# yhtang/GraphDot

Measured on AMD Instinct MI355X. Metric: graph-pairs/sec (Gram matrix), higher is better.
Workload: dtype f64

## Files before the change

### graphdot_amd/csrc/device/mgk_oc.h

```cpp
#ifndef GRAPHDOT_HIP_MGK_OC_H_
#define GRAPHDOT_HIP_MGK_OC_H_
#include "mgk_solver.h"

#ifdef GD_STAMPS
#define GD_OC_STAMP(k) (st_t[k] = __builtin_amdgcn_s_memtime())
#else
#define GD_OC_STAMP(k) ((void)0)
#endif
#ifdef GD_MARKS
#define GD_MARK(name) asm volatile("; GDMARK " #name)
#else
#define GD_MARK(name) ((void)0)
#endif

namespace graphdot {
namespace mgk {

template<int DMAX> struct class_order {
    constexpr static int NC = DMAX + 1, NCP = NC * NC;
    unsigned char d1[NCP], d2[NCP];
    constexpr class_order() : d1{}, d2{} {
        int n = 0;
        for (int p = DMAX * DMAX; p >= 0; --p)
            for (int a = 0; a <= DMAX; ++a)
// ... 229 lines not shown
    }

    __device__ static __forceinline__ graph_header_t load_header(graph_header_t const *ptr, [[maybe_unused]] int &n_orig) {
        if constexpr (QUOT) {
            graph_header_t h = scalar_load(ptr);
            n_orig = (int)((unsigned)h.n_node >> 16);
            h.n_node &= 0xFFFF;
            return h;
        } else {
            return scalar_load(ptr);
        }
    }
    __device__ static __forceinline__ Graph view_graph(char const *image, graph_header_t const &h, [[maybe_unused]] int n_orig) {
        if constexpr (QUOT) return Graph::quotient(image, h, n_orig);
        else return Graph(image, h);
    }

    __device__ static __forceinline__ float cg_ratio(float a, float b) { return a / b; }
    __device__ static __forceinline__ double cg_ratio(double a, double b) {
        double y = __builtin_amdgcn_rcp(b);
        y = __builtin_fma(__builtin_fma(-b, y, 1.0), y, y);
        y = __builtin_fma(__builtin_fma(-b, y, 1.0), y, y);
        return a * y;
    }

    __device__ static __forceinline__ int row_pos(int k, int wv, int lane) {
        return k * T + 64 * ((k & 1) ? W - 1 - wv : wv) + lane;
    }

    struct row_t {
        int i1, i2, rs1, rs2, d1, d2, prod;
    };
    constexpr static int GQU = QUOT ? GU : 1, GQV = QUOT ? GV : 1;
    struct grid_t {
        unsigned a[GU], b[GV];
        unsigned j1[GU], j2[GV];
        unsigned t1[GU], t2[GV];
        bool u[GU], v[GV];
        int row;
    };

    __device__ static __forceinline__ void run(PF const &full, lds_t &lds, real *dyn) {
        P const &prm = common(full);
        const int lane = wave::laneid();
        const int tid = (W == 1) ? lane : (int)threadIdx.x;
        const int wv = (W == 1) ? 0 : uni((int)(threadIdx.x / 64));
        real *const lp = dyn;
        real *const lY = lp + (size_t)prm.u_capacity * C;
        unsigned *const rowmap = reinterpret_cast<unsigned *>(lY + (HAS_Y ? (size_t)Y_REALS : (size_t)0));
        char *const lG1 = reinterpret_cast<char *>(rowmap + NR);
        char *const lG2 = lG1 + prm.g_capacity;
        [[maybe_unused]] real *const lV = reinterpret_cast<real *>(lG2 + prm.g_capacity);
        real *const red0 = lds.red[0], *const red1 = lds.red[1];
        using reduce = alternating_reduce<real, W>;
        using sreduce = alternating_reduce<sreal, W>;
        sreal *const sred0 = reinterpret_cast<sreal *>(red0), *const sred1 = reinterpret_cast<sreal *>(red1);
        const unsigned lY_off = uni((int)lds_offset(lY));
        graph_header_t const *const headers = reinterpret_cast<graph_header_t const *>(prm.arena);
        const int dump = (int)prm.u_capacity - 1;

        if constexpr (DENSE) {
            if (prm.flags & F_DENSE) {
                for (unsigned k = tid; k < prm.u_capacity * (unsigned)C; k += T) lp[k] = real(0);
                job_sync<W>();
            }
        }
#ifdef GD_STAMPS
        unsigned long long st_t[6], st_acc[7] = {0, 0, 0, 0, 0, 0, 0};
#endif
        for (unsigned t = blockIdx.x; t < prm.n_launch_jobs; t += gridDim.x) {
            GD_OC_STAMP(0);
            const job_t job = scalar_load(prm.jobs + t);
            [[maybe_unused]] int no1 = 0, no2 = 0;
            graph_header_t h1 = load_header(headers + job.i, no1), h2 = load_header(headers + job.j, no2);
            if constexpr (ORIENT) {
                bool flip = false;
#pragma unroll
                for (int d = GV + 1; d <= DMAX; ++d) flip |= h2.hist[d] != 0;
                if (flip) {
                    const graph_header_t h = h1;
                    h1 = h2;
                    h2 = h;
                    const int no = no1;
                    no1 = no2;
                    no2 = no;
                }
            }
            const int n1 = h1.n_node, n2 = h2.n_node, N = n1 * n2;
            const int ldp = n2 | 1;
            const real q = prm.q, q0 = prm.q0;
            const real inv1q2 = real(1) / ((real(1) - q) * (real(1) - q));
            const real bscale = q * q / (q0 * q0);
            const unsigned nzpad1 = ((unsigned)n1 + 3u) & ~3u, nzpad2 = ((unsigned)n2 + 3u) & ~3u;
            const unsigned cb1 = TAB ? (nzpad1 + (((unsigned)h1.n_nz + 3u) & ~3u) + 15u) & ~15u : 0u;
            const unsigned cb2 = TAB ? (nzpad2 + (((unsigned)h2.n_nz + 3u) & ~3u) + 15u) & ~15u : 0u;

            GD_MARK(stage);
            job_sync<W>();
            {
                typedef unsigned v4 __attribute__((ext_vector_type(4)));
                const unsigned w1 = (h1.perm + 2u * n1 - h1.degree + cb1 + 15u) / 16u;
                const unsigned w2 = (h2.perm + 2u * n2 - h2.degree + cb2 + 15u) / 16u;
                const v4 *const s1 = reinterpret_cast<const v4 *>(prm.arena + h1.degree - cb1);
                const v4 *const s2 = reinterpret_cast<const v4 *>(prm.arena + h2.degree - cb2);
                v4 *const d1 = reinterpret_cast<v4 *>(lG1);
                v4 *const d2 = reinterpret_cast<v4 *>(lG2);
                constexpr int K = 2;
                const unsigned wmax = w1 > w2 ? w1 : w2;
#pragma nounroll
                for (unsigned base = 0; base < wmax; base += K * T) {
                    v4 v1[K], v2[K];
#pragma unroll
                    for (int k = 0; k < K; ++k) {
                        const unsigned w = base + k * T + tid;
                        v1[k] = w < w1 ? s1[w] : v4{0u, 0u, 0u, 0u};
                        v2[k] = w < w2 ? s2[w] : v4{0u, 0u, 0u, 0u};
                    }
#pragma unroll
                    for (int k = 0; k < K; ++k) {
                        const unsigned w = base + k * T + tid;
                        if (w < w1) d1[w] = v1[k];
                        if (w < w2) d2[w] = v2[k];
                    }
                }
                if constexpr (!STATIC && !FLY) {
#pragma unroll
                    for (int k = 0; k < R; ++k)
#pragma unroll
                        for (int c = 0; c < C; ++c) lY[(k * T + tid) * C + c] = 0;
                }
            }
            const Graph g1 = view_graph(lG1 + cb1 - h1.degree, h1, no1);
            const Graph g2 = view_graph(lG2 + cb2 - h2.degree, h2, no2);
            [[maybe_unused]] auto qweight = [](Graph const &g, nz_t z) -> real {
                return real(at32(g.scale, (unsigned)z.i)) * real(at32(g.scale, (unsigned)z.j));
            };
            std::uint8_t const *const ncls1 = reinterpret_cast<std::uint8_t const *>(lG1);
            std::uint8_t const *const ncls2 = reinterpret_cast<std::uint8_t const *>(lG2);
            std::uint8_t const *const ecls1 = ncls1 + nzpad1;
            std::uint8_t const *const ecls2 = ncls2 + nzpad2;
            const unsigned nvc = prm.n_vclass, nec = prm.n_eclass;
            real const *const kvtab = prm.tables;
            real const *const ketab = kvtab + nvc * nvc;
            real const *const dkvtab = ketab + nec * nec;
            real const *const dketab = dkvtab + (size_t)NodeK::jac_dims * nvc * nvc;
            auto kappa_v = [&](int i1, int i2, node_t const &v1, node_t const &v2) -> real {
                if constexpr (TAB) return at32(kvtab, __umul24((unsigned)ncls1[i1], nvc) + ncls2[i2]);
                else return real(prm.node_kernel(v1, v2));
            };
            std::uint16_t const *const lrp1 = g1.rowptr;
            std::uint16_t const *const lrp2 = g2.rowptr;
            job_sync<W>();

            [[maybe_unused]] bool dense_pair = false;
            [[maybe_unused]] edge_t *dE1 = nullptr, *dE2T = nullptr;
            if constexpr (DENSE) {
                const unsigned n2p = ((unsigned)n2 + 3u) & ~3u;
                const unsigned nn1 = (unsigned)n1 * (unsigned)n1, nn2 = EW * n2p * DSTRIDE;
                dense_pair = (prm.flags & F_DENSE) && n2 <= (int)DSTRIDE &&
                             23u * (unsigned)h1.n_nz * (unsigned)h2.n_nz > 9u * nn1 * (unsigned)n2 * (unsigned)n2;
                dE1 = reinterpret_cast<edge_t *>(lG2 + prm.g_capacity);
                dE2T = reinterpret_cast<edge_t *>(reinterpret_cast<char *>(dE1) + (nn1 * (unsigned)sizeof(edge_t) + 15u) / 16u * 16u);
                if (dense_pair) {
                    edge_t fill1 = at32(g1.edge, 0u), fill2 = at32(g2.edge, 0u);
                    fill1.weight = 0;
                    fill2.weight = 0;
                    unsigned fw[EW];
                    __builtin_memcpy(fw, &fill2, sizeof(edge_t));
                    unsigned *const planes = reinterpret_cast<unsigned *>(dE2T);
                    for (unsigned k = tid; k < nn1; k += T) dE1[k] = fill1;
                    for (unsigned k = tid; k < nn2; k += T) {
// ... 77 lines not shown
                r.rs2 = lrp2[r.i2];
                r.d1 = ok ? (int)lrp1[r.i1 + 1] - r.rs1 : 0;
                r.d2 = ok ? (int)lrp2[r.i2 + 1] - r.rs2 : 0;
                r.prod = r.d1 * r.d2;
                return r;
            };

            struct walk_t {
                unsigned e1, end1, last1, e2, rs2, end2;
                int row;
                __device__ __forceinline__ bool valid() const { return e1 < end1; }
                __device__ __forceinline__ unsigned a() const { return e1 < last1 ? e1 : last1; }
                __device__ __forceinline__ void next() {
                    ++e2;
                    const bool wrap = e2 == end2;
                    e2 = wrap ? rs2 : e2;
                    e1 += wrap ? 1u : 0u;
                }
            };
            auto open_walk = [&](int kb) -> walk_t {
                const row_t r = open_row(kb);
                const bool live = r.prod > 0;
                walk_t w;
                w.e1 = live ? (unsigned)r.rs1 : 0u;
                w.end1 = live ? (unsigned)(r.rs1 + r.d1) : 0u;
                w.last1 = live ? (unsigned)(r.rs1 + r.d1 - 1) : 0u;
                w.rs2 = live ? (unsigned)r.rs2 : 0u;
                w.end2 = live ? (unsigned)(r.rs2 + r.d2) : 1u;
                w.e2 = w.rs2;
                w.row = r.i1 * ldp + r.i2;
                return w;
            };

            auto open_grid = [&](unsigned base, unsigned elem) -> grid_t {
                const row_t r = open_row(0);
                const bool live = r.prod > 0;
                grid_t g;
                g.row = r.i1 * ldp + r.i2;
#pragma unroll
                for (int k = 0; k < GU; ++k) {
                    g.u[k] = k < r.d1;
                    if (k < GV) g.v[k] = k < r.d2;
                    g.a[k] = live ? (unsigned)r.rs1 + (g.u[k] ? (unsigned)k : 0u) : 0u;
                    if (k < GV) g.b[k] = live ? (unsigned)r.rs2 + (g.v[k] ? (unsigned)k : 0u) : 0u;
                    const nz_t z1 = at32(g1.nz, g.a[k]), z2 = at32(g2.nz, k < GV ? g.b[k] : 0u);
                    g.j1[k] = base + __umul24((unsigned)z1.j, (unsigned)ldp) * elem;
                    if (k < GV) g.j2[k] = (unsigned)z2.j * elem;
                    if constexpr (TAB) {
                        g.t1[k] = __umul24((unsigned)ecls1[g.a[k]], nec);
                        if (k < GV) g.t2[k] = (unsigned)ecls2[g.b[k]];
                    }
                }
                return g;
            };

            GD_MARK(slots);
            real val[SA];
            unsigned adr[NADR];
            const unsigned lp_off = lds_offset(lp);
            constexpr unsigned ELEM = CW * sizeof(real);
            unsigned fm[NM];
#pragma unroll
            for (int w = 0; w < NM; ++w) fm[w] = 0;
            int n_slots = 0;
            if constexpr (!FLY) {
                if constexpr (STATIC) {
#pragma unroll
                    for (int k = 0; k < R; ++k)
                        if (k * T < N) n_slots = LAY::T.end[k];
                } else {
#pragma unroll
                for (int k = 0; k < R; ++k) {
                    const int pos = row_pos(k, wv, 0);
                    int trip = 0;
                    if (pos < N) {
                        const unsigned rm = (unsigned)uni((int)rowmap[pos]);
                        const int i1 = (int)(rm >> 16), i2 = (int)(rm & 0xFFFFu);
                        trip = uni(((int)lrp1[i1 + 1] - (int)lrp1[i1]) * ((int)lrp2[i2 + 1] - (int)lrp2[i2]));
                    }
                    if (trip > 0) {
                        n_slots += trip;
                        const int last = n_slots - 1;
#pragma unroll
                        for (int w = 0; w < NM; ++w)
                            if (last / 32 == w) fm[w] |= 1u << (last % 32);
                    }
                }
                n_slots = n_slots > S ? S : n_slots;
                }
                if constexpr (ONE_PASS) {
                    int kb = 0;
                    walk_t cur = G0 ? walk_t{} : open_walk(0);
                    [[maybe_unused]] grid_t grid;
                    [[maybe_unused]] edge_t ge1[GU], ge2[GV];
                    [[maybe_unused]] real gw1[GQU], gw2[GQV];
                    if constexpr (G0 > 0) {
                        grid = open_grid(lp_off, ELEM);
                        if constexpr (QUOT) {
#pragma unroll
                            for (int k = 0; k < GU; ++k) {
                                gw1[k] = qweight(g1, at32(g1.nz, grid.a[k]));
                                if (k < GV) gw2[k] = qweight(g2, at32(g2.nz, grid.b[k]));
                            }
                        }
                        if constexpr (!TAB || (GD_WEIGHTED && edge_weight<edge_t>::value)) {
#pragma unroll
                            for (int k = 0; k < GU; ++k) {
                                ge1[k] = at32(g1.edge, grid.a[k]);
                                if (k < GV) ge2[k] = at32(g2.edge, grid.b[k]);
                            }
                        }
                    }
                    constexpr bool GPRE = QUOT && TAB && G0 > 0 &&
                        !(sizeof(real) == 8 && G0 == 16 && S == 20 && R == 2);
                    [[maybe_unused]] real gtab[GPRE ? G0 : 1];
                    if constexpr (GPRE) {
#pragma unroll
                        for (int s = 0; s < G0; ++s)
                            gtab[s] = at32(ketab, grid.t1[s / GV] + grid.t2[s % GV]);
                    }
    #pragma unroll
                    for (int s = 0; s < S; ++s) {
                        if (s % SETUP_CHUNK == 0) __builtin_amdgcn_sched_barrier(0);
                        if constexpr (GPRE) {
                            if (s < G0 && s % SETUP_CHUNK == 0) {
#pragma unroll
                                for (int u = s; u < s + SETUP_CHUNK && u < G0; ++u)
                                    asm volatile("" : "+v"(gtab[u]));
                            }
                        }
                        real e;
                        bool ok;
                        unsigned col;
                        if (s < G0) {
                            const int gu = s / GV, gv = s % GV;
                            ok = grid.u[gu] && grid.v[gv];
                            if constexpr (TAB) {
                                if constexpr (GPRE) e = gtab[s];
                                else e = at32(ketab, grid.t1[gu] + grid.t2[gv]);
                                if constexpr (GD_WEIGHTED && edge_weight<edge_t>::value)
                                    e *= real(edge_weight<edge_t>::get(ge1[gu])) *
                                         real(edge_weight<edge_t>::get(ge2[gv]));
                            } else {
                                e = prm.edge_kernel(ge1[gu], ge2[gv]);
                            }
                            if constexpr (QUOT) e *= gw1[gu] * gw2[gv];
                            col = ok ? grid.j1[gu] + grid.j2[gv] : lp_off;
                        } else {
                        ok = cur.valid();
                        const unsigned a = cur.a(), b = cur.e2;
                        const nz_t z1 = at32(g1.nz, a), z2 = at32(g2.nz, b);
                        if constexpr (TAB) {
                            e = at32(ketab, __umul24((unsigned)ecls1[a], nec) + ecls2[b]);
                            if constexpr (GD_WEIGHTED && edge_weight<edge_t>::value)
                                e *= real(edge_weight<edge_t>::get(at32(g1.edge, a))) *
                                     real(edge_weight<edge_t>::get(at32(g2.edge, b)));
                        } else {
                            const edge_t e1 = at32(g1.edge, a), e2 = at32(g2.edge, b);
                            e = prm.edge_kernel(e1, e2);
                        }
                        if constexpr (QUOT) e *= qweight(g1, z1) * qweight(g2, z2);
                        col = ok ? __umul24((unsigned)z1.j, (unsigned)ldp) + (unsigned)z2.j : 0u;
                        col = lp_off + col * ELEM;
                        }
                        if (SL > 0 && s >= SREG) {
                            lV[(s - SREG) * T + tid] = ok ? e : real(0);
                        } else {
                            val[s] = ok ? e : real(0);
                        }
                        if constexpr (PACK) {
                            if (s % 2 == 0) adr[s / 2] = col;
                            else adr[s / 2] |= col << 16;
                        } else {
                            adr[s] = col;
                        }
                        if (s % SETUP_CHUNK == SETUP_CHUNK - 1 || s == S - 1) {
#pragma unroll
                            for (int u = s - s % SETUP_CHUNK; u <= s; ++u) {
                                if (SL > 0 && u >= SREG) {
                                    if constexpr (PACK) asm volatile("" : "+v"(adr[u / 2]));
                                    else asm volatile("" : "+v"(adr[u]));
                                } else if constexpr (PACK) asm volatile("" : "+v"(val[u]), "+v"(adr[u / 2]));
                                else asm volatile("" : "+v"(val[u]), "+v"(adr[u]));
                            }
                        }
                        if (s >= G0) cur.next();
                        if (flush_at(s, fm) && s != S - 1) {
                            ++kb;
                            cur = open_walk(kb);
                        }
                    }
                } else {
                    int kb = 0, j = 0, ja = 0, jb = 0;
                    row_t cur = open_row(0);
                    [[maybe_unused]] unsigned ab_[PACK ? SA : 1];
                    unsigned (&ab)[PACK ? SA : NADR] = select_array<PACK>(ab_, adr);
    #pragma unroll
                    for (int s = 0; s < S; ++s) {
                        ab[s] = (s < n_slots && j < cur.prod)
                            ? ((unsigned)(cur.rs1 + ja) << 16) | (unsigned)(cur.rs2 + jb) : ~0u;
                        asm volatile("" : "+v"(ab[s]));
                        ++j;
                        ++jb;
                        if (jb >= cur.d2) {
                            jb = 0;
                            ++ja;
                        }
                        if ((fm[s / 32] >> (s % 32)) & 1u) {
                            ++kb;
// ... 1171 lines not shown
```

### graphdot_amd/csrc/gdhost.cpp

```cpp
#include "gdhost.h"
#include "gdquotient.h"

#include <algorithm>
#include <cstdlib>
#include <cstring>
#include <numeric>
#include <atomic>
#include <cmath>
#include <exception>
#include <mutex>
#include <thread>
#include <vector>

namespace {

constexpr int64_t ALIGN = 16;
inline int64_t pad(int64_t n) { return (n + ALIGN - 1) / ALIGN * ALIGN; }

struct rect_order_t {
    int a[256], b[256], prod[257];
    int n_upto[16], upto[16][256];
    rect_order_t() {
        int n = 0;
        for (int p = 15 * 15; p >= 0; --p)
// ... 568 lines not shown
        }
    const bool with_jobs = jobs && jobs_sorted;
    parallel_ranges(n_jobs, T, [&](int64_t t0, int64_t t1, int k) {
        std::vector<int64_t> &pos = start[(size_t)k];
        for (int64_t t = t0; t < t1; ++t) {
            const int64_t at = pos[rank[(size_t)t]]++;
            order[at] = (uint32_t)t;
            if (with_jobs) {
                jobs_sorted[2 * at] = jobs[2 * t];
                jobs_sorted[2 * at + 1] = jobs[2 * t + 1];
            }
        }
    });
    return 0;
} catch (...) { return -3; }

int gdh_gather_section(const uint8_t *blob, const int64_t *blob_off, const int64_t *sec_off,
                       int32_t col, const int64_t *count, int64_t G, int32_t itemsize,
                       uint8_t *out, int64_t out_bytes) try {
    if (G < 0 || col < 0 || col >= 6 || itemsize < 0) return -1;
    int64_t at = 0;
    for (int64_t g = 0; g < G; ++g) {
        const int64_t nb = count[g] * (int64_t)itemsize;
        if (nb < 0 || at + nb > out_bytes) return -2;
        std::memcpy(out + at, blob + blob_off[g] + sec_off[g * 6 + col], (size_t)nb);
        at += nb;
    }
    return 0;
} catch (...) { return -3; }

int gdh_assemble_arena(int64_t G, const uint8_t *blob, const int64_t *blob_off,
                       const int64_t *starts, const int64_t *cbytes, const int64_t *n_node,
                       const int64_t *n_nz, const uint8_t *ncls, const uint8_t *ecls,
                       uint8_t *host, int64_t host_bytes) try {
    if (G < 0) return -1;
    int64_t vn = 0, ve = 0;
    for (int64_t g = 0; g < G; ++g) {
        const int64_t nb = blob_off[g + 1] - blob_off[g];
        if (nb < 0 || starts[g] < cbytes[g] || starts[g] + nb > host_bytes) return -2;
        std::memcpy(host + starts[g], blob + blob_off[g], (size_t)nb);
        if (ncls && ecls && cbytes[g] > 0) {
            uint8_t *c0 = host + starts[g] - cbytes[g];
            const int64_t npad = (n_node[g] + 3) / 4 * 4;
            if (npad + n_nz[g] > cbytes[g]) return -2;
            std::memcpy(c0, ncls + vn, (size_t)n_node[g]);
            std::memcpy(c0 + npad, ecls + ve, (size_t)n_nz[g]);
        }
        vn += n_node[g];
        ve += n_nz[g];
    }
    return 0;
} catch (...) { return -3; }

int gdh_pairwise_jobs(int64_t nx, int64_t ny, uint32_t *jobs) try {
    if (nx < 0 || ny < -1 || nx + (ny > 0 ? ny : 0) > 0xFFFFFFFFll) return -1;
    int64_t t = 0;
    if (ny < 0) {
        for (int64_t i = 0; i < nx; ++i)
            for (int64_t j = i; j < nx; ++j, ++t) {
                jobs[2 * t] = (uint32_t)i;
                jobs[2 * t + 1] = (uint32_t)j;
            }
    } else {
        for (int64_t i = 0; i < nx; ++i)
            for (int64_t j = 0; j < ny; ++j, ++t) {
                jobs[2 * t] = (uint32_t)i;
                jobs[2 * t + 1] = (uint32_t)(nx + j);
            }
    }
    return 0;
} catch (...) { return -3; }

}
```

### graphdot_amd/hip/hostlib.py

```python
import ctypes
import os
import subprocess
import threading
import numpy as np

_HERE = os.path.dirname(os.path.abspath(__file__))
CSRC = os.path.join(os.path.dirname(_HERE), 'csrc')
INCLUDE = os.path.join(os.path.dirname(os.path.dirname(_HERE)), 'include')
LIB_PATH = os.path.join(CSRC, 'libgdhost.so')
_lock = threading.Lock()
_lib = None

_vp, _i32, _i64 = ctypes.c_void_p, ctypes.c_int32, ctypes.c_int64
SIGNATURES = {
    'gdh_pack_graphs': [_i32] + [_vp] * 7 + [_i32, _vp, _i32, _i32, _i32, _i32,
                                            _vp, _i64] + [_vp] * 10
    + [_i64, _vp, _vp],
    'gdh_number_records': [_vp, _i64, _i32, _vp, _vp, _i32, _vp, _vp, _vp],
    'gdh_classify_oc': [_i64] + [_vp] * 7 + [_i32] + [_vp] * 6
    + [_i32, _i32, _i64, _i32, _vp, _vp, _vp],
    'gdh_pair_keys': [_vp, _i64, _vp, _i32, _i32, _vp, _vp],
    'gdh_order_jobs': [_vp, _i64, _vp, _i64, _i64, _vp, _vp, _vp],
    'gdh_pairwise_jobs': [_i64, _i64, _vp],
    'gdh_gather_section': [_vp, _vp, _vp, _i32, _vp, _i64, _i32, _vp, _i64],
    'gdh_assemble_arena': [_i64] + [_vp] * 9 + [_i64],
    'gdh_quotient_graph': [_i32, _i32, _vp, _vp, _i32, _vp, _vp, _vp, _i32,
                           _vp, _vp, _i64, _vp, _vp],
}


class HostLibError(RuntimeError):
    pass


def build_library(force=False):
    src = os.path.join(CSRC, 'gdhost.cpp')
    hdrs = [os.path.join(INCLUDE, h) for h in ('gdhost.h', 'gdquotient.h')]
    if (not force and os.path.exists(LIB_PATH)
            and os.path.getmtime(LIB_PATH) >= max(
                os.path.getmtime(f) for f in [src] + hdrs)):
        return LIB_PATH
    cxx = os.environ.get('CXX', 'g++')
    tmp = LIB_PATH + f'.{os.getpid()}.tmp'
    cmd = [cxx, '-O2', '-fPIC', '-shared', '-std=c++17', '-pthread',
           f'-I{INCLUDE}', src,
           '-o', tmp]
    r = subprocess.run(cmd, capture_output=True, text=True)
    if r.returncode != 0:
        raise HostLibError(f'building libgdhost.so failed:\n{r.stderr}')
    os.replace(tmp, LIB_PATH)
    return LIB_PATH


def lib():
    global _lib
    with _lock:
        if _lib is None:
            L = ctypes.CDLL(build_library())
# ... 132 lines not shown
    raw = out = None
    if jobs is not None:
        jobs = np.ascontiguousarray(jobs)
        raw = jobs.view(np.uint32)
        out = np.empty_like(jobs)
    _check(lib().gdh_order_jobs(
        _p(pk), len(pk), _p(rank_of_key), len(rank_of_key), int(n_ranks),
        _p(order), _p(raw), None if out is None else _p(out.view(np.uint32))),
        'gdh_order_jobs')
    return order if jobs is None else (order, out)


def pairwise_jobs(nx, ny=None, dtype=None):
    n = nx * (nx + 1) // 2 if ny is None else nx * ny
    jobs = np.empty(2 * n, np.uint32)
    _check(lib().gdh_pairwise_jobs(int(nx), -1 if ny is None else int(ny),
                                   _p(jobs)), 'gdh_pairwise_jobs')
    return jobs if dtype is None else jobs.view(dtype)


def gather_section(blob, blob_off, sec_off, col, count, dtype):
    dtype = np.dtype(dtype)
    count = _c(count, np.int64)
    blob_off = _c(blob_off, np.int64)
    out = np.empty(int(count.sum()), dtype=dtype)
    raw = out.view(np.uint8) if dtype.itemsize else out
    _check(lib().gdh_gather_section(
        _p(blob), _p(blob_off), _p(_c(sec_off, np.int64)), int(col), _p(count),
        len(count), dtype.itemsize, _p(raw), out.nbytes), 'gdh_gather_section')
    return out


def assemble_arena(blob, blob_off, starts, cbytes, n_node, n_nz, ncls, ecls,
                   host):
    _check(lib().gdh_assemble_arena(
        len(starts), _p(blob), _p(_c(blob_off, np.int64)),
        _p(_c(starts, np.int64)), _p(_c(cbytes, np.int64)),
        _p(_c(n_node, np.int64)), _p(_c(n_nz, np.int64)),
        None if ncls is None else _p(_c(ncls, np.uint8)),
        None if ecls is None else _p(_c(ecls, np.uint8)),
        _p(host), host.nbytes), 'gdh_assemble_arena')


def quotient_graph(dg):
    n, nnz = int(dg.n_node), int(dg.n_nz)
    nsz, esz = np.dtype(dg.node_t).itemsize, np.dtype(dg.edge_t).itemsize
    o, src = dg.offsets, np.ascontiguousarray(dg.blob)
    base = src.ctypes.data

    def at(name):
        return ctypes.c_void_p(base + int(o[name]))
    cap = len(src) + 8 * n + 64
    blob = np.empty(cap, np.uint8)
    offs = np.zeros(7, np.int64)
    counts = np.zeros(3, np.int64)
    _check(lib().gdh_quotient_graph(
        n, nnz, at('degree'), at('node'), nsz, at('rowptr'), at('nz'),
        at('edge'), esz, at('perm'), _p(blob), cap, _p(offs), _p(counts)),
        'gdh_quotient_graph')
    return blob[:int(counts[2])], offs.tolist(), int(counts[0]), int(counts[1])


_collect = None


def collector():
    global _collect
    if _collect is None:
        with _lock:
            if _collect is None:
                _collect = _build_collector()
    return _collect

# ... 61 lines not shown
```

### graphdot_amd/kernel/marginalized/_backend_hip.py

```python
import copy
import os
import re
import uuid
import zlib
from collections import OrderedDict, namedtuple
import numpy as np
from ...codegen import Template
from ...util import gcpause
from ...util.cookie import IdentityCache
from ...codegen.sympy_printer import to_real_expr
from ...codegen.typetool import _dtype_util
from ...hip import jit, runtime
from ...microkernel import TensorProduct, Product
from ...util.iterable import flatten, fold_like
from ._backend import Backend
from ._devicegraph import (DeviceGraph, GraphArena, HIST_BINS, class_bytes,
                           degree_histograms, graph_features, pack_many,
                           quotient_graph)

_TEMPLATE = os.path.join(os.path.dirname(__file__), 'template.hip')

F_NODAL, F_DIAGONAL, F_SYMMETRIC, F_LMIN1, F_BLOCK, F_PACKED, F_REFCOMPAT, \
    F_DENSE = 1, 2, 4, 8, 16, 32, 64, 128

Variant = namedtuple('Variant', 'W S R')
OCVariant = namedtuple('OCVariant', 'W S R D L', defaults=(None,))


STREAM_PART_EFFICIENCY = ((1, 1.0), (2, 0.74), (4, 0.58), (8, 0.53),
                          (16, 0.50), (32, 0.49), (64, 0.46), (128, 0.35),
                          (256, 0.26))


def stream_parts(costs, count, resident, queued):
    if costs is None or len(costs) == 0:
        return max(1, min(resident // max(count, 1), STREAM_MAX_PARTS))
    c = np.asarray(costs, dtype=np.float64)
    best, best_t = 1, max(c[0], c.sum() / max(1, min(resident, queued)))
    table = dict(STREAM_PART_EFFICIENCY)
    ms, es = zip(*STREAM_PART_EFFICIENCY)
    own = min(resident // max(len(c), 1), STREAM_MAX_PARTS)
    for M in sorted(set(ms[1:]) | ({own} if own > 1 else set())):
        if M > min(resident, STREAM_MAX_PARTS):
            break
        eff = table.get(M) or float(np.interp(np.log2(M), np.log2(ms), es))
        groups = max(1, resident // M)
        pad = -len(c) % groups
        load = np.concatenate((c, np.zeros(pad))).reshape(-1, groups).sum(0)
        t = load.max() / (M * eff)
# ... 426 lines not shown
    @staticmethod
    def _assert_homogeneous(x, y):
        if (x.weighted != y.weighted or x.node_t != y.node_t
                or x.edge_t != y.edge_t):
            raise TypeError(
                'All nodes/edges must be of the same type: '
                f'{x.node_t} / {x.edge_t} vs {y.node_t} / {y.edge_t}. '
                'If the graph attributes match in name but differ in type, '
                'try to normalize automatically with '
                '`Graph.unify_datatype`.')

    @staticmethod
    def _used_fields(kernel):
        fun, jac = kernel.gen_expr('x1', 'x2')
        text = ' '.join([fun, *jac])
        names = set(re.findall(r'\bx[12]\.([A-Za-z_]\w*)', text))
        bare = re.search(r'\bx[12]\b(?!\.[A-Za-z_])', text)
        return None if bare else tuple(sorted(names))

    def _table_bytes(self, arena):
        c = arena.classes
        if self.tables != 'lds' or c is None:
            return 0
        b = (c['nv']**2 + c['ne']**2) * np.dtype(self.real).itemsize
        return int(-(-b // 16) * 16) if b <= TABLE_LDS_LIMIT else 0

    def _global_tables(self, arena):
        c = arena.classes
        return (self.tables == 'global' and c is not None
                and c['nv']**2 + c['ne']**2 <= GLOBAL_TABLE_LIMIT)

    def _host_arena(self, dgraphs, fields):
        return GraphArena(dgraphs, *fields, classes=bool(self.tables),
                          native=self.native)

    def _arena(self, dgraphs, fields=(None, None)):
        key = (_ids(dgraphs), fields if self.tables else None)
        hit = self._arenas.get(key)
        if hit is not None:
            self._arenas.move_to_end(key)
            return hit
        arena = self._host_arena(dgraphs, fields)
        buf = runtime.DeviceBuffer(arena.nbytes)
        buf.upload(arena.relocated(buf.ptr))
        runtime.synchronize()
        self._arenas[key] = (arena, buf, list(dgraphs))
        while len(self._arenas) > 4:
            self._arenas.popitem(last=False)
        return self._arenas[key]

    @staticmethod
    def gencode_kernel(kernel, name, real=np.float32):
        fun, jac = kernel.gen_expr('x1', 'x2')
        rn = _real_name(real)
        fun = to_real_expr(fun, np.dtype(real).name)
        jac = [to_real_expr(j, np.dtype(real).name) for j in jac]
        return Template(r'''
${theta_t}
struct ${name}_t : ${name}_theta_t {
    constexpr static int jac_dims = ${jac_dims};
    template<class X> __device__ __forceinline__
    auto operator() (X const &x1, X const &x2) const {
        return ${expr};
    }
    template<class X> __device__ __forceinline__
    auto _j_a_c_o_b_i_a_n_(X const &x1, X const &x2) const {
        graphdot::array<real_t, jac_dims> j;
# ... 581 lines not shown
        H, hid = self._degree_hists(dgraphs, maxdeg, D, hists)
        nH = len(H)
        row = np.full(len(ji), -1, dtype=np.int64)
        idx = np.flatnonzero(pair_maxdeg <= D)
        pk = hid[ji[idx]] * nH + hid[jj[idx]]
        upk, inv = np.unique(pk, return_inverse=True)
        row[idx] = inv.reshape(-1)
        tr = self.oc_trips(H[upk // nH], H[upk % nH], D, self.TRIP_BATCHES)
        return tr, row

    def _classify_pairs(self, ji, jj, dgraphs, C, tab_bytes=0, gtab=False,
                        oc_only=False, nodal=False, mfma=False):
        f = graph_features(dgraphs)
        n_node, n_nz = f['n_node'], f['n_nz']
        deg_sorted = None
        n1, n2 = n_node[ji], n_node[jj]
        nnz1 = n_nz[ji]
        N = n1 * n2
        NP = n1 * (n2 | 1)
        NP_either = np.maximum(NP, n2 * (n1 | 1))

        def rows_of(v):
            g = self.grid_of(v.L, v.D) if isinstance(v, OCVariant) else None
            return NP_either if g is not None and g[0] != g[1] else NP
        cost = n_nz[ji] * n_nz[jj] + 4 * N
        choice = np.full(len(ji), -1, dtype=np.int64)
        slots = {}
        ntask = np.maximum((nnz1 + 1) * n2, n1 + n2 + 2)
        image = f['image_bytes']
        if tab_bytes:
            image = image + class_bytes(n_node, n_nz)
        gbytes = np.maximum(image[ji], image[jj])
        image_oc = image + class_bytes(n_node, n_nz) if gtab else image
        gbytes_oc = np.maximum(image_oc[ji], image_oc[jj])
        maxdeg = f['max_degree']
        pair_maxdeg = np.maximum(maxdeg[ji], maxdeg[jj])
        oc_slots, hists, trips = {}, {}, {}
        fly_off = False
        rem = np.arange(len(ji))
        is_oc = [isinstance(v, OCVariant) for v in self.variants]
        n_oc = sum(is_oc)
        quot = bool(C == 1 and not nodal and len(dgraphs) and
                    getattr(dgraphs[0], 'n_orig', None) is not None)

        def grid_fits(v, idx):
            g = self.grid_of(v.L, v.D)
            if g is None:
                return np.ones(len(idx), dtype=bool)
            a, b = maxdeg[ji[idx]], maxdeg[jj[idx]]
            return (np.maximum(a, b) <= g[0]) & (np.minimum(a, b) <= g[1])
        menu = [(k, v) for k, v in enumerate(self.variants[:n_oc])
                if isinstance(v, OCVariant)
                and (not v.L or self._static_enabled(v, C, quot))
                and (v.S > 0 or not fly_off)]
        native_oc = (self.native and not tab_bytes and n_oc > 0
                     and all(is_oc[:n_oc]) and len(ji) > 0
                     and len(dgraphs) < 2**31)
        if native_oc:
            from ...hip import hostlib
            hist = f['hist']
            ch, _ = hostlib.classify_oc(
                ji, jj, n_node, n_nz, image_oc, maxdeg, hist,
                [(v.W, v.S, v.R, v.D, v.L) for _, v in menu], C,
                np.dtype(self.real).itemsize, LDS_LIMIT, FLY_MIN_DEGREE,
                [self.lds_slot_bytes(v, C, nodal) for _, v in menu])
            idx = np.array([k for k, _ in menu], dtype=np.int64)
# ... 1004 lines not shown
```

### graphdot_amd/kernel/marginalized/_devicegraph.py

```python
import itertools as it
import numpy as np
from operator import itemgetter
from numpy.lib.recfunctions import repack_fields
from ...codegen.cpptool import cpptype
from ...codegen.typetool import common_min_type, is_scalar_type

_ALIGN = 16

HEADER_DTYPE = np.dtype([
    ('n_node', np.int32), ('n_nz', np.int32), ('degree', np.uint32),
    ('node', np.uint32), ('rowptr', np.uint32), ('nz', np.uint32),
    ('edge', np.uint32), ('perm', np.uint32), ('hist', np.uint16, (16,))],
    align=True)
assert HEADER_DTYPE.itemsize == 64
HIST_BINS = 16


def degree_histogram(adjacency_count):
    c = np.minimum(np.asarray(adjacency_count, dtype=np.int64), HIST_BINS - 1)
    return np.bincount(c, minlength=HIST_BINS).astype(np.uint16)
SECTIONS = ('degree', 'node', 'rowptr', 'nz', 'edge', 'perm')

NZ_DTYPE = np.dtype([('i', np.uint16), ('j', np.uint16)])

# ... 693 lines not shown

def quotient_graph(dg, native=True):
    if len(dg.relocs):
        return None
    if native:
        from ...hip import hostlib
        blob, offs, nq, nnz = hostlib.quotient_graph(dg)
    else:
        blob, offs, nq, nnz = _quotient_blob_numpy(dg)
    q = DeviceGraph.__new__(DeviceGraph)
    q.n_node, q.n_nz, q.n_orig, q.weighted = nq, nnz, dg.n_node, dg.weighted
    q.node_t, q.edge_t, q.signature = dg.node_t, dg.edge_t, dg.signature
    q.offsets = dict(zip(QUOTIENT_SECTIONS, offs))
    o = q.offsets
    q.blob = blob
    q.degree = blob[o['degree']:o['degree'] + 4 * nq].view(np.float32)
    q.scale = blob[o['scale']:o['scale'] + 8 * nq].view(np.float64)
    q.rowptr = blob[o['rowptr']:o['rowptr'] + 2 * (nq + 1)].view(np.uint16)
    q.nz = blob[o['nz']:o['nz'] + 4 * nnz].view(NZ_DTYPE)
    q.perm = blob[o['perm']:o['perm'] + 2 * nq].view(np.uint16)
    q.adjacency_count = np.diff(q.rowptr.astype(np.int64))
    q.image_bytes = _pad(o['perm'] + 2 * nq)
    q.relocs = np.zeros(0, dtype=np.int64)
    q.n_merged = dg.n_node - nq
    return q


def class_bytes(n_node, n_nz):
    n_node, n_nz = np.asarray(n_node), np.asarray(n_nz)
    return ((n_node + 3) // 4 * 4 + (n_nz + 3) // 4 * 4 + _ALIGN - 1) \
        // _ALIGN * _ALIGN


def _label_classes(dgraphs, vfields=None, efields=None, max_classes=255,
                   native=True):
    if not dgraphs or any(len(g.relocs) for g in dgraphs):
        return None
    g0 = dgraphs[0]
    node_t, edge_t = np.dtype(g0.node_t), np.dtype(g0.edge_t)

    def number(records, fields):
        dt = records.dtype
        if fields is not None:
            if not set(fields) <= set(dt.names or ()):
                return None
            keys = records[sorted(fields)] if fields else None
            if keys is not None:
                keys = repack_fields(keys)
        else:
            keys = records if dt.itemsize else None
        if keys is None or len(records) == 0 or keys.dtype.itemsize == 0:
            return np.zeros(len(records), np.int64), records[:1]
        if native:
            from ...hip import hostlib
            parts = [(0, dt.itemsize)] if fields is None else \
                [(dt.fields[f][1], dt.fields[f][0].itemsize)
                 for f in sorted(fields)]
            inv, first = hostlib.number_records(records, parts)
            rec = np.ascontiguousarray(records).view(np.uint8).reshape(
                len(records), dt.itemsize)[first]
            return inv.astype(np.int64), \
                np.ascontiguousarray(rec).view(dt).reshape(-1)
        raw = np.ascontiguousarray(keys).view(np.uint8).reshape(
            len(keys), keys.dtype.itemsize)
        if raw.shape[1] <= 8:
            wide = np.zeros((len(raw), 8), dtype=np.uint8)
# ... 33 lines not shown
    nodes = gather('node', feat['n_node'].tolist(), node_t)
    edges = gather('edge', feat['n_nz'].tolist(), edge_t)
    numbered = number(nodes, vfields)
    if numbered is None:
        return None
    ncls, vrep = numbered
    if g0.weighted:
        label_t = edge_t.fields['label'][0]
        numbered = number(np.ascontiguousarray(edges['label']), efields)
        if numbered is None:
            return None
        ecls, lrep = numbered
        erep = np.zeros(max(len(lrep), 1), dtype=edge_t)
        erep['weight'] = 1
        if label_t.itemsize and len(lrep):
            erep['label'] = lrep
    else:
        numbered = number(edges, efields)
        if numbered is None:
            return None
        ecls, erep = numbered
        if len(erep) == 0:
            erep = np.zeros(1, dtype=edge_t)
    if len(vrep) == 0:
        vrep = np.zeros(1, dtype=node_t)
    if len(vrep) > max_classes or len(erep) > max_classes:
        return None
    return ncls.astype(np.uint8), ecls.astype(np.uint8), vrep, erep


class GraphArena:

    def __init__(self, dgraphs, vfields=None, efields=None, classes=True,
                 native=True):
        self.n = len(dgraphs)
        hdr_bytes = _pad(self.n * HEADER_DTYPE.itemsize)
        cls = _label_classes(dgraphs, vfields, efields, native=native) \
            if classes else None
        self.classes = None
        cursor = hdr_bytes
        if cls is not None:
            ncls, ecls, vrep, erep = cls
            self.classes = dict(nv=len(vrep), ne=len(erep), vrep=cursor,
                                erep=cursor + _pad(vrep.nbytes))
            cursor = self.classes['erep'] + _pad(erep.nbytes)
        feat = graph_features(dgraphs) if self.n else None
        b0 = whole_batch(dgraphs)
        sizes = np.diff(np.asarray(b0['blob_off'], dtype=np.int64)) \
            if b0 is not None else np.array([len(g.blob) for g in dgraphs],
                                            dtype=np.int64)
        cbytes = class_bytes(feat['n_node'], feat['n_nz']) \
            if self.n else np.zeros(0, np.int64)
        ends = cursor + np.cumsum(sizes + cbytes)
        starts = ends - sizes if self.n else np.zeros(0, np.int64)
        self.nbytes = int(ends[-1]) if self.n else int(cursor)
        self.host = np.zeros(self.nbytes, dtype=np.uint8)
        self.blob_start = starts
        self.class_bytes = cbytes
        if cls is not None:
            c = self.classes
            self.host[c['vrep']:c['vrep'] + vrep.nbytes] = \
                vrep.view(np.uint8).ravel() if vrep.nbytes else []
            self.host[c['erep']:c['erep'] + erep.nbytes] = \
                erep.view(np.uint8).ravel() if erep.nbytes else []
        self._relocs = []
        hdr = np.zeros(self.n, dtype=HEADER_DTYPE)
        natively = native and b0 is not None and self.n > 0
        if natively:
            from ...hip import hostlib
            hostlib.assemble_arena(
                b0['blob'], b0['blob_off'], starts, cbytes, feat['n_node'],
                feat['n_nz'], None if cls is None else ncls,
                None if cls is None else ecls, self.host)
        elif b0 is not None and not cbytes.any():
            self.host[cursor:] = b0['blob']
        elif b0 is not None:
            host, blob, bo = self.host, b0['blob'], b0['blob_off']
            for k, s in enumerate(starts.tolist()):
                host[s:s + bo[k + 1] - bo[k]] = blob[bo[k]:bo[k + 1]]
        else:
            for g, s in zip(dgraphs, starts.tolist()):
                self.host[s:s + len(g.blob)] = g.blob
                if len(g.relocs):
                    self._relocs.append(g.relocs + s)
                    words = self.host
                    for where in g.relocs + s:
                        word = words[where:where + 8].view(np.uint64)
                        word[0] += np.uint64(s)
        if self.n:
            n_node, n_nz = feat['n_node'], feat['n_nz']
            hdr['n_node'], hdr['n_nz'] = n_node, n_nz
            if getattr(dgraphs[0], 'n_orig', None) is not None:
                hdr['n_node'] = (n_node | (np.array(
                    [g.n_orig for g in dgraphs], dtype=np.int64) << 16)
                ).astype(np.uint32).view(np.int32)
            for s_, name in enumerate(SECTIONS):
                hdr[name] = starts + (
                    b0['sec_off'][:, s_] if b0 is not None else np.array(
                        [g.offsets[name] for g in dgraphs], dtype=np.int64))
            hdr['hist'] = feat['hist']
            if cls is not None and not natively:
                c0 = starts - cbytes
                node0 = np.cumsum(n_node) - n_node
                self.host[np.repeat(c0 - node0, n_node)
                          + np.arange(int(n_node.sum()))] = ncls
                c1 = c0 + (n_node + 3) // 4 * 4
                nz0 = np.cumsum(n_nz) - n_nz
                self.host[np.repeat(c1 - nz0, n_nz)
                          + np.arange(int(n_nz.sum()))] = ecls
        self._hdr = hdr
        self._relocs = (np.concatenate(self._relocs) if self._relocs
                        else np.zeros(0, np.int64))
        self.n_node = hdr['n_node'].astype(np.int64) & 0xFFFF
        self.n_nz = hdr['n_nz'].astype(np.int64)

    def relocated(self, base):
        if self.nbytes >= 2**32:
            raise ValueError('graph arena exceeds the 4 GiB offset range')
        img = self.host.copy()
        img[:self._hdr.nbytes] = self._hdr.view(np.uint8)
        for where in self._relocs:
            word = img[where:where + 8].view(np.uint64)
            word[0] += np.uint64(base)
        return img
```

### include/gdhost.h

```cpp
#ifndef GDHOST_H_
#define GDHOST_H_

#include <stddef.h>
#include <stdint.h>

#ifdef __cplusplus
extern "C" {
#endif

const char *gdh_version(void);

int gdh_pack_graphs(int32_t G, const int64_t *node_off, const int64_t *edge_off,
                    const int64_t *node_id, const int64_t *ei, const int64_t *ej,
                    const float *w, const uint8_t *node_rec, int32_t node_size,
                    const uint8_t *label_rec, int32_t label_size,
                    int32_t edge_size, int32_t label_offset, int32_t weight_bytes,
                    uint8_t *blob, int64_t blob_capacity, int64_t *blob_off,
                    int64_t *sec_off, int64_t *nnz, uint16_t *perm, int64_t *rank,
                    float *degree, int64_t *count, uint16_t *rowptr, uint16_t *nz,
                    int64_t *eid, int64_t nz_capacity, int64_t *nz_off,
                    int64_t *maxdeg);

int gdh_number_records(const uint8_t *rec, int64_t n, int32_t itemsize,
                       const int32_t *part_off, const int32_t *part_len,
                       int32_t n_parts, int32_t *cls, int64_t *first,
                       int64_t *n_classes);

int gdh_classify_oc(int64_t n_pairs, const int32_t *ca, const int32_t *cb,
                    const int32_t *n_node, const int32_t *n_nz,
                    const int64_t *image_bytes, const int32_t *maxdeg,
                    const uint16_t *hist, int32_t n_var, const int32_t *W,
                    const int32_t *S, const int32_t *R, const int32_t *D,
                    const int32_t *n_L, const int32_t *L, int32_t C,
                    int32_t real_size, int64_t lds_limit, int32_t fly_min_degree,
                    const int64_t *extra_lds, int32_t *choice, int64_t *NP);

int gdh_pair_keys(const uint32_t *jobs, int64_t n_jobs, const int32_t *cid,
                  int32_t n_graphs, int32_t nc, int32_t *pk, int64_t *count);

int gdh_order_jobs(const int32_t *pk, int64_t n_jobs, const int32_t *rank_of_key,
                   int64_t n_keys, int64_t n_ranks, uint32_t *order,
                   const uint32_t *jobs, uint32_t *jobs_sorted);

int gdh_gather_section(const uint8_t *blob, const int64_t *blob_off, const int64_t *sec_off,
                       int32_t col, const int64_t *count, int64_t G, int32_t itemsize,
                       uint8_t *out, int64_t out_bytes);

int gdh_assemble_arena(int64_t G, const uint8_t *blob, const int64_t *blob_off,
                       const int64_t *starts, const int64_t *cbytes, const int64_t *n_node,
                       const int64_t *n_nz, const uint8_t *ncls, const uint8_t *ecls,
                       uint8_t *host, int64_t host_bytes);

int gdh_pairwise_jobs(int64_t nx, int64_t ny, uint32_t *jobs);

#ifdef __cplusplus
}
#endif
#endif
```

Before: 251.6 million.

## Precompute packed per-edge term records in arena for quotient-graph f64 kernels

Adds a 16-byte per-edge record (qw=scale_i*scale_j, weight, column j, edge class) built on the host and staged into LDS before the class and graph data. The kernel's grid and walk setup then reads one vector load per edge instead of gathering the nz entry, two scale values and the edge class separately. This cuts scattered LDS reads and multiplies, and masking of setup values is deferred to the end of each chunk. In exchange, each pair copies more bytes into LDS, which raises LDS footprint and may lower occupancy or push some pairs onto a different path.

```diff
diff --git a/graphdot_amd/csrc/device/mgk_oc.h b/graphdot_amd/csrc/device/mgk_oc.h
--- a/graphdot_amd/csrc/device/mgk_oc.h
+++ b/graphdot_amd/csrc/device/mgk_oc.h
@@ -285,6 +285,14 @@
         int i1, i2, rs1, rs2, d1, d2, prod;
     };
     constexpr static int GQU = QUOT ? GU : 1, GQV = QUOT ? GV : 1;
+    constexpr static bool RECS = QUOT && TAB && ONE_PASS && sizeof(real) == 8;
+    typedef unsigned term_t __attribute__((ext_vector_type(4)));
+    __device__ static __forceinline__ double term_qw(term_t const &t) {
+        const unsigned long long bits = ((unsigned long long)t.y << 32) | t.x;
+        return __builtin_bit_cast(double, bits);
+    }
+    __device__ static __forceinline__ unsigned term_j(term_t const &t) { return t.w & 0xFFFFu; }
+    __device__ static __forceinline__ unsigned term_cls(term_t const &t) { return (t.w >> 16) & 0xFFu; }
     struct grid_t {
         unsigned a[GU], b[GV];
         unsigned j1[GU], j2[GV];
@@ -347,15 +355,17 @@
             const unsigned nzpad1 = ((unsigned)n1 + 3u) & ~3u, nzpad2 = ((unsigned)n2 + 3u) & ~3u;
             const unsigned cb1 = TAB ? (nzpad1 + (((unsigned)h1.n_nz + 3u) & ~3u) + 15u) & ~15u : 0u;
             const unsigned cb2 = TAB ? (nzpad2 + (((unsigned)h2.n_nz + 3u) & ~3u) + 15u) & ~15u : 0u;
+            const unsigned tb1 = RECS ? 16u * (unsigned)h1.n_nz : 0u, tb2 = RECS ? 16u * (unsigned)h2.n_nz : 0u;
+            const unsigned pre1 = cb1 + tb1, pre2 = cb2 + tb2;
 
             GD_MARK(stage);
             job_sync<W>();
             {
                 typedef unsigned v4 __attribute__((ext_vector_type(4)));
-                const unsigned w1 = (h1.perm + 2u * n1 - h1.degree + cb1 + 15u) / 16u;
-                const unsigned w2 = (h2.perm + 2u * n2 - h2.degree + cb2 + 15u) / 16u;
-                const v4 *const s1 = reinterpret_cast<const v4 *>(prm.arena + h1.degree - cb1);
-                const v4 *const s2 = reinterpret_cast<const v4 *>(prm.arena + h2.degree - cb2);
+                const unsigned w1 = (h1.perm + 2u * n1 - h1.degree + pre1 + 15u) / 16u;
+                const unsigned w2 = (h2.perm + 2u * n2 - h2.degree + pre2 + 15u) / 16u;
+                const v4 *const s1 = reinterpret_cast<const v4 *>(prm.arena + h1.degree - pre1);
+                const v4 *const s2 = reinterpret_cast<const v4 *>(prm.arena + h2.degree - pre2);
                 v4 *const d1 = reinterpret_cast<v4 *>(lG1);
                 v4 *const d2 = reinterpret_cast<v4 *>(lG2);
                 constexpr int K = 2;
@@ -383,13 +393,15 @@
                         for (int c = 0; c < C; ++c) lY[(k * T + tid) * C + c] = 0;
                 }
             }
-            const Graph g1 = view_graph(lG1 + cb1 - h1.degree, h1, no1);
-            const Graph g2 = view_graph(lG2 + cb2 - h2.degree, h2, no2);
+            const Graph g1 = view_graph(lG1 + pre1 - h1.degree, h1, no1);
+            const Graph g2 = view_graph(lG2 + pre2 - h2.degree, h2, no2);
+            [[maybe_unused]] term_t const *const terms1 = reinterpret_cast<term_t const *>(lG1);
+            [[maybe_unused]] term_t const *const terms2 = reinterpret_cast<term_t const *>(lG2);
             [[maybe_unused]] auto qweight = [](Graph const &g, nz_t z) -> real {
                 return real(at32(g.scale, (unsigned)z.i)) * real(at32(g.scale, (unsigned)z.j));
             };
-            std::uint8_t const *const ncls1 = reinterpret_cast<std::uint8_t const *>(lG1);
-            std::uint8_t const *const ncls2 = reinterpret_cast<std::uint8_t const *>(lG2);
+            std::uint8_t const *const ncls1 = reinterpret_cast<std::uint8_t const *>(lG1) + tb1;
+            std::uint8_t const *const ncls2 = reinterpret_cast<std::uint8_t const *>(lG2) + tb2;
             std::uint8_t const *const ecls1 = ncls1 + nzpad1;
             std::uint8_t const *const ecls2 = ncls2 + nzpad2;
             const unsigned nvc = prm.n_vclass, nec = prm.n_eclass;
@@ -533,7 +545,8 @@
                 return w;
             };
 
-            auto open_grid = [&](unsigned base, unsigned elem) -> grid_t {
+            auto open_grid = [&](unsigned base, unsigned elem, [[maybe_unused]] real *qw1 = nullptr,
+                                 [[maybe_unused]] real *qw2 = nullptr) -> grid_t {
                 const row_t r = open_row(0);
                 const bool live = r.prod > 0;
                 grid_t g;
@@ -544,6 +557,18 @@
                     if (k < GV) g.v[k] = k < r.d2;
                     g.a[k] = live ? (unsigned)r.rs1 + (g.u[k] ? (unsigned)k : 0u) : 0u;
                     if (k < GV) g.b[k] = live ? (unsigned)r.rs2 + (g.v[k] ? (unsigned)k : 0u) : 0u;
+                    if constexpr (RECS) {
+                        const term_t r1 = at32(terms1, g.a[k]), r2 = at32(terms2, k < GV ? g.b[k] : 0u);
+                        g.j1[k] = base + __umul24(term_j(r1), (unsigned)ldp) * elem;
+                        g.t1[k] = __umul24(term_cls(r1), nec);
+                        qw1[k] = term_qw(r1);
+                        if (k < GV) {
+                            g.j2[k] = term_j(r2) * elem;
+                            g.t2[k] = term_cls(r2);
+                            qw2[k] = term_qw(r2);
+                        }
+                        continue;
+                    }
                     const nz_t z1 = at32(g1.nz, g.a[k]), z2 = at32(g2.nz, k < GV ? g.b[k] : 0u);
                     g.j1[k] = base + __umul24((unsigned)z1.j, (unsigned)ldp) * elem;
                     if (k < GV) g.j2[k] = (unsigned)z2.j * elem;
@@ -595,9 +620,11 @@
                     [[maybe_unused]] grid_t grid;
                     [[maybe_unused]] edge_t ge1[GU], ge2[GV];
                     [[maybe_unused]] real gw1[GQU], gw2[GQV];
+                    [[maybe_unused]] bool wok[SETUP_CHUNK];
                     if constexpr (G0 > 0) {
-                        grid = open_grid(lp_off, ELEM);
-                        if constexpr (QUOT) {
+                        if constexpr (RECS) grid = open_grid(lp_off, ELEM, gw1, gw2);
+                        else grid = open_grid(lp_off, ELEM);
+                        if constexpr (QUOT && !RECS) {
 #pragma unroll
                             for (int k = 0; k < GU; ++k) {
                                 gw1[k] = qweight(g1, at32(g1.nz, grid.a[k]));
@@ -650,6 +677,16 @@
                         } else {
                         ok = cur.valid();
                         const unsigned a = cur.a(), b = cur.e2;
+                        if constexpr (RECS) {
+                            const term_t r1 = at32(terms1, a), r2 = at32(terms2, b);
+                            e = at32(ketab, __umul24(term_cls(r1), nec) + term_cls(r2));
+                            if constexpr (GD_WEIGHTED && edge_weight<edge_t>::value)
+                                e *= real(edge_weight<edge_t>::get(at32(g1.edge, a))) *
+                                     real(edge_weight<edge_t>::get(at32(g2.edge, b)));
+                            e *= term_qw(r1) * term_qw(r2);
+                            col = ok ? __umul24(term_j(r1), (unsigned)ldp) + term_j(r2) : 0u;
+                            col = lp_off + col * ELEM;
+                        } else {
                         const nz_t z1 = at32(g1.nz, a), z2 = at32(g2.nz, b);
                         if constexpr (TAB) {
                             e = at32(ketab, __umul24((unsigned)ecls1[a], nec) + ecls2[b]);
@@ -664,8 +701,12 @@
                         col = ok ? __umul24((unsigned)z1.j, (unsigned)ldp) + (unsigned)z2.j : 0u;
                         col = lp_off + col * ELEM;
                         }
+                        }
                         if (SL > 0 && s >= SREG) {
                             lV[(s - SREG) * T + tid] = ok ? e : real(0);
+                        } else if (RECS && s >= G0) {
+                            val[s] = e;
+                            wok[s % SETUP_CHUNK] = ok;
                         } else {
                             val[s] = ok ? e : real(0);
                         }
@@ -676,6 +717,15 @@
                             adr[s] = col;
                         }
                         if (s % SETUP_CHUNK == SETUP_CHUNK - 1 || s == S - 1) {
+                            if constexpr (RECS) {
+#pragma unroll
+                                for (int u = s - s % SETUP_CHUNK; u <= s; ++u) {
+                                    if (u >= G0 && !(SL > 0 && u >= SREG)) {
+                                        asm volatile("" : "+v"(val[u]));
+                                        val[u] = wok[u % SETUP_CHUNK] ? val[u] : real(0);
+                                    }
+                                }
+                            }
 #pragma unroll
                             for (int u = s - s % SETUP_CHUNK; u <= s; ++u) {
                                 if (SL > 0 && u >= SREG) {
diff --git a/graphdot_amd/csrc/gdhost.cpp b/graphdot_amd/csrc/gdhost.cpp
--- a/graphdot_amd/csrc/gdhost.cpp
+++ b/graphdot_amd/csrc/gdhost.cpp
@@ -624,8 +624,13 @@
 int gdh_assemble_arena(int64_t G, const uint8_t *blob, const int64_t *blob_off,
                        const int64_t *starts, const int64_t *cbytes, const int64_t *n_node,
                        const int64_t *n_nz, const uint8_t *ncls, const uint8_t *ecls,
-                       uint8_t *host, int64_t host_bytes) try {
+                       const int64_t *term_off, int32_t edge_size, int32_t weight_off,
+                       int32_t weight_size, uint8_t *host, int64_t host_bytes) try {
     if (G < 0) return -1;
+    if (term_off && (!ncls || !ecls || edge_size < 0 ||
+                     (weight_off >= 0 && ((weight_size != 4 && weight_size != 8) ||
+                                          weight_off + weight_size > edge_size))))
+        return -1;
     int64_t vn = 0, ve = 0;
     for (int64_t g = 0; g < G; ++g) {
         const int64_t nb = blob_off[g + 1] - blob_off[g];
@@ -638,6 +643,41 @@
             std::memcpy(c0, ncls + vn, (size_t)n_node[g]);
             std::memcpy(c0 + npad, ecls + ve, (size_t)n_nz[g]);
         }
+        if (term_off) {
+            const int64_t nz_n = n_nz[g], first = starts[g] - cbytes[g] - 16 * nz_n;
+            const int64_t *off = term_off + 3 * g;
+            if (first < 0 || off[0] < 0 || off[1] < 0 || off[2] < 0 ||
+                off[0] + 8 * n_node[g] > nb || off[1] + 4 * nz_n > nb ||
+                off[2] + (int64_t)edge_size * nz_n > nb)
+                return -2;
+            const uint8_t *src = blob + blob_off[g];
+            uint8_t *out = host + first;
+            for (int64_t e = 0; e < nz_n; ++e, out += 16) {
+                uint16_t ij[2];
+                std::memcpy(ij, src + off[1] + 4 * e, 4);
+                if (ij[0] >= n_node[g] || ij[1] >= n_node[g]) return -2;
+                double si, sj;
+                std::memcpy(&si, src + off[0] + 8 * (int64_t)ij[0], 8);
+                std::memcpy(&sj, src + off[0] + 8 * (int64_t)ij[1], 8);
+                const double q = si * sj;
+                float w = 1.0f;
+                if (weight_off >= 0) {
+                    const uint8_t *rec = src + off[2] + (int64_t)edge_size * e + weight_off;
+                    if (weight_size == 4) {
+                        std::memcpy(&w, rec, 4);
+                    } else {
+                        double wd;
+                        std::memcpy(&wd, rec, 8);
+                        w = (float)wd;
+                    }
+                }
+                const uint8_t tail[2] = {ecls[ve + e], 0};
+                std::memcpy(out, &q, 8);
+                std::memcpy(out + 8, &w, 4);
+                std::memcpy(out + 12, &ij[1], 2);
+                std::memcpy(out + 14, tail, 2);
+            }
+        }
         vn += n_node[g];
         ve += n_nz[g];
     }
diff --git a/graphdot_amd/hip/hostlib.py b/graphdot_amd/hip/hostlib.py
--- a/graphdot_amd/hip/hostlib.py
+++ b/graphdot_amd/hip/hostlib.py
@@ -23,7 +23,7 @@
     'gdh_order_jobs': [_vp, _i64, _vp, _i64, _i64, _vp, _vp, _vp],
     'gdh_pairwise_jobs': [_i64, _i64, _vp],
     'gdh_gather_section': [_vp, _vp, _vp, _i32, _vp, _i64, _i32, _vp, _i64],
-    'gdh_assemble_arena': [_i64] + [_vp] * 9 + [_i64],
+    'gdh_assemble_arena': [_i64] + [_vp] * 9 + [_i32] * 3 + [_vp, _i64],
     'gdh_quotient_graph': [_i32, _i32, _vp, _vp, _i32, _vp, _vp, _vp, _i32,
                            _vp, _vp, _i64, _vp, _vp],
 }
@@ -222,13 +222,22 @@
 
 
 def assemble_arena(blob, blob_off, starts, cbytes, n_node, n_nz, ncls, ecls,
-                   host):
+                   host, term_off=None, edge_t=None):
+    edge_size, weight_off, weight_size = 0, -1, 0
+    if term_off is not None:
+        edge_t = np.dtype(edge_t)
+        edge_size = edge_t.itemsize
+        if edge_t.names and 'weight' in edge_t.names:
+            weight_off = edge_t.fields['weight'][1]
+            weight_size = edge_t.fields['weight'][0].itemsize
     _check(lib().gdh_assemble_arena(
         len(starts), _p(blob), _p(_c(blob_off, np.int64)),
         _p(_c(starts, np.int64)), _p(_c(cbytes, np.int64)),
         _p(_c(n_node, np.int64)), _p(_c(n_nz, np.int64)),
         None if ncls is None else _p(_c(ncls, np.uint8)),
         None if ecls is None else _p(_c(ecls, np.uint8)),
+        None if term_off is None else _p(_c(term_off, np.int64)),
+        edge_size, weight_off, weight_size,
         _p(host), host.nbytes), 'gdh_assemble_arena')
 
 
diff --git a/graphdot_amd/kernel/marginalized/_backend_hip.py b/graphdot_amd/kernel/marginalized/_backend_hip.py
--- a/graphdot_amd/kernel/marginalized/_backend_hip.py
+++ b/graphdot_amd/kernel/marginalized/_backend_hip.py
@@ -15,6 +15,7 @@
 from ...util.iterable import flatten, fold_like
 from ._backend import Backend
 from ._devicegraph import (DeviceGraph, GraphArena, HIST_BINS, class_bytes,
+                           term_bytes,
                            degree_histograms, graph_features, pack_many,
                            quotient_graph)
 
@@ -507,7 +508,8 @@
 
     def _host_arena(self, dgraphs, fields):
         return GraphArena(dgraphs, *fields, classes=bool(self.tables),
-                          native=self.native)
+                          native=self.native,
+                          terms=np.dtype(self.real) == np.float64)
 
     def _arena(self, dgraphs, fields=(None, None)):
         key = (_ids(dgraphs), fields if self.tables else None)
@@ -1155,6 +1157,9 @@
             image = image + class_bytes(n_node, n_nz)
         gbytes = np.maximum(image[ji], image[jj])
         image_oc = image + class_bytes(n_node, n_nz) if gtab else image
+        if (gtab and np.dtype(self.real) == np.float64 and len(dgraphs)
+                and getattr(dgraphs[0], 'n_orig', None) is not None):
+            image_oc = image_oc + term_bytes(n_nz)
         gbytes_oc = np.maximum(image_oc[ji], image_oc[jj])
         maxdeg = f['max_degree']
         pair_maxdeg = np.maximum(maxdeg[ji], maxdeg[jj])
diff --git a/graphdot_amd/kernel/marginalized/_devicegraph.py b/graphdot_amd/kernel/marginalized/_devicegraph.py
--- a/graphdot_amd/kernel/marginalized/_devicegraph.py
+++ b/graphdot_amd/kernel/marginalized/_devicegraph.py
@@ -749,6 +749,14 @@
         // _ALIGN * _ALIGN
 
 
+TERM_DTYPE = np.dtype([('qw', np.float64), ('w', np.float32),
+                       ('j', np.uint16), ('cls', np.uint8), ('pad', np.uint8)])
+
+
+def term_bytes(n_nz):
+    return np.asarray(n_nz) * TERM_DTYPE.itemsize
+
+
 def _label_classes(dgraphs, vfields=None, efields=None, max_classes=255,
                    native=True):
     if not dgraphs or any(len(g.relocs) for g in dgraphs):
@@ -848,7 +856,7 @@
 class GraphArena:
 
     def __init__(self, dgraphs, vfields=None, efields=None, classes=True,
-                 native=True):
+                 native=True, terms=True):
         self.n = len(dgraphs)
         hdr_bytes = _pad(self.n * HEADER_DTYPE.itemsize)
         cls = _label_classes(dgraphs, vfields, efields, native=native) \
@@ -867,12 +875,17 @@
                                             dtype=np.int64)
         cbytes = class_bytes(feat['n_node'], feat['n_nz']) \
             if self.n else np.zeros(0, np.int64)
-        ends = cursor + np.cumsum(sizes + cbytes)
+        with_terms = bool(terms and cls is not None and self.n and getattr(
+            dgraphs[0], 'n_orig', None) is not None)
+        tbytes = term_bytes(feat['n_nz']) if with_terms \
+            else np.zeros(self.n, np.int64)
+        ends = cursor + np.cumsum(sizes + cbytes + tbytes)
         starts = ends - sizes if self.n else np.zeros(0, np.int64)
         self.nbytes = int(ends[-1]) if self.n else int(cursor)
         self.host = np.zeros(self.nbytes, dtype=np.uint8)
         self.blob_start = starts
         self.class_bytes = cbytes
+        self.term_bytes = tbytes
         if cls is not None:
             c = self.classes
             self.host[c['vrep']:c['vrep'] + vrep.nbytes] = \
@@ -881,8 +894,18 @@
                 erep.view(np.uint8).ravel() if erep.nbytes else []
         self._relocs = []
         hdr = np.zeros(self.n, dtype=HEADER_DTYPE)
-        natively = native and b0 is not None and self.n > 0
-        if natively:
+        natively = native and self.n > 0 and (b0 is not None or with_terms)
+        if natively and with_terms:
+            from ...hip import hostlib
+            hostlib.assemble_arena(
+                np.concatenate([g.blob for g in dgraphs]),
+                np.concatenate(([0], np.cumsum(sizes))), starts, cbytes,
+                feat['n_node'], feat['n_nz'], ncls, ecls, self.host,
+                term_off=np.array(
+                    [[g.offsets[s] for s in ('scale', 'nz', 'edge')]
+                     for g in dgraphs], dtype=np.int64),
+                edge_t=dgraphs[0].edge_t)
+        elif natively:
             from ...hip import hostlib
             hostlib.assemble_arena(
                 b0['blob'], b0['blob_off'], starts, cbytes, feat['n_node'],
@@ -924,6 +947,21 @@
                 nz0 = np.cumsum(n_nz) - n_nz
                 self.host[np.repeat(c1 - nz0, n_nz)
                           + np.arange(int(n_nz.sum()))] = ecls
+                if with_terms:
+                    edge_t = np.dtype(dgraphs[0].edge_t)
+                    for k, g in enumerate(dgraphs):
+                        rec = np.zeros(g.n_nz, dtype=TERM_DTYPE)
+                        zi, zj = g.nz['i'].astype(np.int64), g.nz['j']
+                        rec['qw'] = g.scale[zi] * g.scale[zj.astype(np.int64)]
+                        rec['w'] = 1
+                        if g.weighted:
+                            o = g.offsets['edge']
+                            rec['w'] = g.blob[o:o + g.n_nz * edge_t.itemsize] \
+                                .view(edge_t)['weight']
+                        rec['j'] = zj
+                        rec['cls'] = ecls[nz0[k]:nz0[k] + g.n_nz]
+                        at = int(c0[k] - tbytes[k])
+                        self.host[at:at + rec.nbytes] = rec.view(np.uint8)
         self._hdr = hdr
         self._relocs = (np.concatenate(self._relocs) if self._relocs
                         else np.zeros(0, np.int64))
diff --git a/include/gdhost.h b/include/gdhost.h
--- a/include/gdhost.h
+++ b/include/gdhost.h
@@ -49,7 +49,8 @@
 int gdh_assemble_arena(int64_t G, const uint8_t *blob, const int64_t *blob_off,
                        const int64_t *starts, const int64_t *cbytes, const int64_t *n_node,
                        const int64_t *n_nz, const uint8_t *ncls, const uint8_t *ecls,
-                       uint8_t *host, int64_t host_bytes);
+                       const int64_t *term_off, int32_t edge_size, int32_t weight_off,
+                       int32_t weight_size, uint8_t *host, int64_t host_bytes);
 
 int gdh_pairwise_jobs(int64_t nx, int64_t ny, uint32_t *jobs);
 
```

After: 258.8 million, median of 6. 1.03x the previous value.
